# OpenIFEM/OpenIFEM

Hardware: AMD Instinct MI355X
Metric: DoF/s per Newton step (assemble+solve), 3D INS Q2/Q1 (higher is better)
Workload: dtype f64; 1 GPU; 3D channel flow 128x128x128 Q2/Q1, mpi_insim Newton step (plane Poiseuille + seeded 1e-3 perturbation), 128^3 cells per GPU; n_dofs=53070468, cells_per_gpu=2097152, parallelism=dd1, fgmres_iters=1, inner_iters=4, cg_mp_iters=0, cg_sm_iters=2, rccl_nranks=0, comm_transport=none (single rank), halo_neighbors=0

## Files before the change

### __graft_entry__.py

```python
import os
import subprocess
import sys

ROOT = os.path.dirname(os.path.abspath(__file__))
sys.path.insert(0, ROOT)
sys.path.insert(0, os.path.join(ROOT, "tests"))


def build():
    jobs = str(min(8, os.cpu_count() or 1))
    subprocess.check_call(["make", "-C", os.path.join(ROOT, "openifem_amd", "csrc"), "-j", jobs])
    subprocess.check_call(["make", "-C", os.path.join(ROOT, "oracle")])
    import openifem_amd.capi as capi
    L = capi.load()
    missing = [s for s in capi.EXPORTS + capi.EXPORTS_SA_WALL if not hasattr(L, s)]
    if missing:
        raise RuntimeError(f"libifem_hip.so lacks symbols: {missing}")


def smoke():
    import numpy as np
    import openifem_amd.capi as capi
    import orc
    from boxmesh import BoxMesh
    from cases import channel3d_state

    m = BoxMesh([4, 4, 4], (0, 0, 0), (2.0, 0.2, 0.2), kv=2)
    dofs, vals, present, evalp, kw = channel3d_state(m)
    ctx = capi.Context(3, 2, m.vcoords, m.cell_unodes, m.cell_pnodes, m.cell_face_bid, m.n_unodes, m.n_pnodes)
    ctx.set_constraints(0, dofs, None)
    ctx.set_constraints(1, dofs, vals)
    ctx.vec_set(capi.VEC_PRESENT, present)
    ctx.vec_set(capi.VEC_EVAL, evalp)
    P = capi.make_params(**kw)
    ctx.opts.ainv_kind = 3
    ctx.assemble(P, False)
    st = ctx.solve(P, False)
    upd = ctx.vec_get(capi.VEC_UPDATE)
# ... 18 lines not shown
```

### include/ifem_hip_testing.h

```cpp
#ifndef IFEM_HIP_TESTING_H
#define IFEM_HIP_TESTING_H
#include "ifem_hip.h"
#ifdef __cplusplus
extern "C" {
#endif

int ifem_tpp_ilu_probe(ifem_ctx *ctx, int64_t *rowptr, int32_t *col, double *val, const double *x, double *y, int32_t *levels);
int ifem_tpp_override(ifem_ctx *ctx, const double *val);

int ifem_scns_pc_probe(ifem_ctx *ctx, int which, const double *x, double *y);

int ifem_test_restart_fits(ifem_ctx *ctx, int columns);

int ifem_test_mf_uniform(ifem_ctx *ctx, double *h);

int ifem_test_asm_rows(ifem_ctx *ctx, int verbose, int32_t *state);

int ifem_test_uu_vmult_f32col(ifem_ctx *ctx, int dst, int src);

int ifem_test_uu_patch_vmult(ifem_ctx *ctx, int dst, int src);
int ifem_test_uu_patch_info(ifem_ctx *ctx, int64_t out[4]);

enum {
  IFEM_TVK_MDOT = 0, IFEM_TVK_MDOT_SELF, IFEM_TVK_MAXPY, IFEM_TVK_MAXPY_NORM, IFEM_TVK_MDOT_F32, IFEM_TVK_MAXPY_F32, IFEM_TVK_MAXPY_F32_NORM,
  IFEM_TVK_SCALE_STORE_F32, IFEM_TVK_AXPY, IFEM_TVK_AXPBY, IFEM_TVK_SCALE_TO2, IFEM_TVK_DIV, IFEM_TVK_MINMAX, IFEM_TVK_COUNT
};
int ifem_test_vec_kernel(ifem_ctx *ctx, int op, int64_t n, int k, int64_t ld, void *V, const double *coef, double *w, double *out);

int ifem_test_cg_device(ifem_ctx *ctx, int64_t n, const double *a, const double *jac, const double *b, int iters, double *x);

int ifem_test_uu_fused_product(ifem_ctx *ctx, int prec, int mode, int first, double a, double b, const double *x, double *xs, double *r, double *d,
                               int block_cap, int64_t geo[2]);

enum { IFEM_TMG_PAD = 8 };
int ifem_test_mg_transfer(ifem_ctx *ctx, int kind, int64_t n_rows, int64_t n_cols, const int64_t *ptr, const int32_t *col, const double *w,
                          const uint8_t *flag_in, const uint8_t *flag_out, const double *x, double *y);

int ifem_test_mg_lattice_transfer(ifem_ctx *fine, int which, int path, const double *x, double *y, int64_t info[4]);

// ... 20 lines not shown
```

### openifem_amd/capi.py

```python
import ctypes as C
import os

import numpy as np

_HERE = os.path.dirname(os.path.abspath(__file__))
os.environ.setdefault("HSA_ENABLE_IPC_MODE_LEGACY", "0")
LIB_PATH = os.path.join(_HERE, "lib", "libifem_hip.so")

VEC_PRESENT, VEC_EVAL, VEC_FSI_ACC, VEC_UPDATE, VEC_RHS, VEC_INCREMENT, VEC_TMP = range(7)
E_BADPARAM, E_NODEVICE, E_HIP, E_KRYLOV_NOCONV, E_NEWTON_MAXIT, E_COMM = -1, -2, -3, -4, -5, -6
E_NODEVICE_EXIT = 66
AINV_GMRES_BJACOBI, AINV_GMRES_BJACOBI_F32, AINV_SCALAR_GMRES, AINV_GMRES_BJACOBI_MF, AINV_MG = range(5)


class MeshDesc(C.Structure):
    _fields_ = [("dim", C.c_int32), ("kv", C.c_int32), ("n_cells", C.c_int32),
                ("n_unodes_owned", C.c_int32), ("n_unodes_local", C.c_int32),
                ("n_pnodes_owned", C.c_int32), ("n_pnodes_local", C.c_int32),
                ("vcoords", C.c_void_p), ("cell_unodes", C.c_void_p), ("cell_pnodes", C.c_void_p),
                ("cell_face_bid", C.c_void_p)]


class Partition(C.Structure):
    _fields_ = [("rank", C.c_int32), ("nranks", C.c_int32), ("n_neighbors", C.c_int32),
# ... 123 lines not shown
           "ifem_set_cell_fields", "ifem_vec_set", "ifem_vec_get", "ifem_vec_copy", "ifem_vec_zero", "ifem_vec_axpy",
           "ifem_vec_norm2", "ifem_vec_minmax", "ifem_halo_exchange", "ifem_ins_assemble", "ifem_solve",
           "ifem_rhs_norm", "ifem_ins_newton_step", "ifem_system_vmult", "ifem_uu_vmult", "ifem_precond_vmult", "ifem_export_csr",
           "ifem_get_timing", "ifem_set_profiling", "ifem_synchronize", "ifem_set_hanging_constraints", "ifem_set_ainv_kind", "ifem_set_scns_fields", "ifem_update_stress",
           "ifem_scns_assemble", "ifem_scns_solve", "ifem_scns_newton_step", "ifem_imex_assemble", "ifem_imex_solve",
           "ifem_imex_step", "ifem_set_eddy_viscosity", "ifem_default_tuning", "ifem_set_tuning", "ifem_abi_sizeof",
           "ifem_mass_vmult", "ifem_mg_attach", "ifem_mg_depth", "ifem_uu_block_diag",
           "ifem_fsi_set_solid", "ifem_fsi_update_indicator", "ifem_fsi_find_fluid_bc", "ifem_fsi_get_stress",
           "ifem_get_constraints", "ifem_fsi_fluid_at_points", "ifem_comm_stats_get", "ifem_comm_stats_level", "ifem_true_residual", "ifem_tpp_ilu_probe", "ifem_tpp_override", "ifem_scns_pc_probe", "ifem_test_restart_fits",
           "ifem_kprof_begin", "ifem_kprof_end", "ifem_kprof_family_name", "ifem_export_rows", "ifem_export_uu_pattern", "ifem_vcycle_graph_stats", "ifem_inner_restart_length",
           "ifem_uu_stored_bytes", "ifem_test_mf_uniform", "ifem_test_asm_rows", "ifem_test_uu_vmult_f32col",
           "ifem_test_uu_patch_vmult", "ifem_test_uu_patch_info", "ifem_test_vec_kernel", "ifem_test_cg_device",
           "ifem_test_uu_fused_product", "ifem_test_mp_solve", "ifem_test_sm_apply", "ifem_test_b_apply", "ifem_test_sm_solve",
           "ifem_test_mg_transfer", "ifem_test_mg_vec_kernel", "ifem_test_mg_lattice_transfer",
           "ifem_sa_set_wall_points", "ifem_sa_get_wall_distance", "ifem_sa_set_constraints", "ifem_sa_vec_set", "ifem_sa_vec_get",
           "ifem_sa_assemble", "ifem_sa_solve", "ifem_sa_newton_step", "ifem_sa_update_eddy_viscosity", "ifem_sa_export_csr",
           "ifem_scnsex_setup", "ifem_scnsex_assemble_rhs", "ifem_scnsex_solve", "ifem_scnsex_step", "ifem_scnsex_export_csr",
           "ifem_kelly_estimate", "ifem_transfer_solution"]
FACE_BOUNDARY, FACE_EQUAL, FACE_COARSER, FACE_FINER = range(4)

EXPORTS_SA_WALL = ["ifem_sa_set_moving_wall", "ifem_sa_set_shear_velocities", "ifem_sa_update_shear_velocity", "ifem_sa_get_shear_velocity", "ifem_sa_update_moving_wall_distance",
                   "ifem_sa_get_moving_wall", "ifem_sa_update_boundary_condition", "ifem_sa_get_constraints"]
SA_NO_MOVING_WALL = np.finfo(float).max

SM_CG, SM_MG, SM_DIRECT = 0, 1, 2

(TVK_MDOT, TVK_MDOT_SELF, TVK_MAXPY, TVK_MAXPY_NORM, TVK_MDOT_F32, TVK_MAXPY_F32, TVK_MAXPY_F32_NORM, TVK_SCALE_STORE_F32, TVK_AXPY,
 TVK_AXPBY, TVK_SCALE_TO2, TVK_DIV, TVK_MINMAX) = range(13)

(TMG_CHEB_INIT, TMG_CHEB_STEP, TMG_VEC_RECIP, TMG_VEC_ROUGH, TMG_CVT_D2F, TMG_CVT_F2D, TMG_AXPY_F32V, TMG_VC_EXIT, TMG_VC_EXIT_F32,
 TMG_INJECT_NODES, TMG_VC_ENTRY, TMG_VC_ENTRY_F32, TMG_CHEB_INIT_BLOCK_F32) = range(13)
TMG_PAD = 8

ABI_STRUCTS = None

_lib = None


class IfemError(RuntimeError):
    def __init__(self, code, msg):
        super().__init__(f"ifem error {code}: {msg}")
        self.code = code


def load():
    global _lib
# ... 48 lines not shown
    L.ifem_set_ainv_kind.argtypes = [C.c_void_p, C.c_int]
    L.ifem_set_scns_fields.argtypes = [C.c_void_p, C.c_void_p, C.c_void_p, C.c_void_p]
    L.ifem_set_eddy_viscosity.argtypes = [C.c_void_p, C.c_void_p]
    L.ifem_update_stress.argtypes = [C.c_void_p, C.c_double, C.c_void_p]
    L.ifem_scns_assemble.argtypes = [C.c_void_p, C.POINTER(ScnsParams), C.c_int]
    L.ifem_imex_assemble.argtypes = [C.c_void_p, C.POINTER(InsParams), C.c_int, C.c_int]
    L.ifem_imex_solve.argtypes = [C.c_void_p, C.POINTER(InsParams), C.POINTER(SolverOpts), C.c_int, C.POINTER(SolveStats)]
    L.ifem_imex_step.argtypes = [C.c_void_p, C.POINTER(InsParams), C.POINTER(SolverOpts), C.c_int, C.c_int, C.POINTER(SolveStats)]
    L.ifem_scns_solve.argtypes = [C.c_void_p, C.POINTER(SolverOpts), C.c_int, C.POINTER(SolveStats)]
    L.ifem_scns_newton_step.argtypes = [C.c_void_p, C.POINTER(ScnsParams), C.POINTER(SolverOpts), C.c_int, C.c_double,
                                        C.c_int, C.c_void_p]
    L.ifem_default_tuning.argtypes = [C.POINTER(Tuning)]
    L.ifem_set_tuning.argtypes = [C.c_void_p, C.POINTER(Tuning)]
    L.ifem_mg_attach.argtypes = [C.c_void_p, C.c_void_p, C.POINTER(MgTransfer)]
    L.ifem_mg_depth.argtypes = [C.c_void_p]
    L.ifem_comm_stats_get.argtypes = [C.c_void_p, C.c_void_p, C.c_int]
    L.ifem_comm_stats_level.argtypes = [C.c_void_p, C.c_int, C.c_void_p]
    L.ifem_tpp_ilu_probe.argtypes = [C.c_void_p] + [C.c_void_p] * 6
    L.ifem_tpp_override.argtypes = [C.c_void_p, C.c_void_p]
    L.ifem_scns_pc_probe.argtypes = [C.c_void_p, C.c_int, C.c_void_p, C.c_void_p]
    L.ifem_test_restart_fits.argtypes = [C.c_void_p, C.c_int]
    L.ifem_test_mf_uniform.argtypes = [C.c_void_p, C.c_void_p]
    L.ifem_test_asm_rows.argtypes = [C.c_void_p, C.c_int, C.c_void_p]
    L.ifem_test_uu_vmult_f32col.argtypes = [C.c_void_p, C.c_int, C.c_int]
    L.ifem_test_uu_patch_vmult.argtypes = [C.c_void_p, C.c_int, C.c_int]
    L.ifem_test_uu_patch_info.argtypes = [C.c_void_p, C.c_void_p]
    L.ifem_test_vec_kernel.argtypes = [C.c_void_p, C.c_int, C.c_int64, C.c_int, C.c_int64, C.c_void_p, C.c_void_p, C.c_void_p, C.c_void_p]
    L.ifem_test_cg_device.argtypes = [C.c_void_p, C.c_int64, C.c_void_p, C.c_void_p, C.c_void_p, C.c_int, C.c_void_p]
    L.ifem_test_uu_fused_product.argtypes = [C.c_void_p, C.c_int, C.c_int, C.c_int, C.c_double, C.c_double, C.c_void_p, C.c_void_p, C.c_void_p,
                                             C.c_void_p, C.c_int, C.c_void_p]
    L.ifem_test_mp_solve.argtypes = [C.c_void_p, C.POINTER(SolverOpts), C.c_void_p, C.c_void_p, C.c_void_p]
    L.ifem_test_sm_apply.argtypes = [C.c_void_p, C.c_int, C.c_void_p, C.c_void_p, C.c_void_p]
    L.ifem_test_sm_solve.argtypes = [C.c_void_p, C.POINTER(SolverOpts), C.c_void_p, C.c_void_p, C.c_void_p]
    L.ifem_test_b_apply.argtypes = [C.c_void_p, C.c_int, C.c_int, C.c_void_p, C.c_void_p, C.c_void_p]
    L.ifem_test_mg_transfer.argtypes = [C.c_void_p, C.c_int, C.c_int64, C.c_int64] + [C.c_void_p] * 7
    L.ifem_test_mg_lattice_transfer.argtypes = [C.c_void_p, C.c_int, C.c_int, C.c_void_p, C.c_void_p, C.c_void_p]
    L.ifem_test_mg_vec_kernel.argtypes = [C.c_void_p, C.c_int, C.c_int64, C.c_int64] + [C.c_void_p] * 7
    L.ifem_true_residual.argtypes = [C.c_void_p, C.POINTER(C.c_double), C.POINTER(C.c_double)]
    L.ifem_kprof_begin.argtypes = [C.c_void_p]
    L.ifem_kprof_end.argtypes = [C.c_void_p, C.c_void_p, C.c_int32]
    L.ifem_kprof_family_name.argtypes = [C.c_int32]
    L.ifem_kprof_family_name.restype = C.c_char_p
    L.ifem_uu_block_diag.argtypes = [C.c_void_p, C.c_int, C.c_void_p]
    L.ifem_fsi_set_solid.argtypes = [C.c_void_p, C.POINTER(FsiSolid)]
    L.ifem_fsi_update_indicator.argtypes = [C.c_void_p, C.c_void_p, C.POINTER(C.c_int64)]
    L.ifem_fsi_find_fluid_bc.argtypes = [C.c_void_p, C.c_double, C.c_int, C.c_void_p, C.POINTER(FsiStats)]
# ... 294 lines not shown
    def __del__(self):
        try:
            self.close()
        except Exception:
            pass

    def set_tuning(self, **kw):
        t = Tuning()
        self.L.ifem_default_tuning(C.byref(t))
        if getattr(self, "_tuning", None) is not None:
            t = self._tuning
        for k, v in kw.items():
            if not hasattr(t, k):
                raise AttributeError(k)
            setattr(t, k, v)
        self._chk(self.L.ifem_set_tuning(self.h, C.byref(t)))
        self._tuning = t

    def asm_rows_state(self, verbose=False):
        st = C.c_int32(0)
        self._chk(self.L.ifem_test_asm_rows(self.h, int(verbose), C.byref(st)))
        return int(st.value)

    def uu_stored_bytes(self):
        return int(self.L.ifem_uu_stored_bytes(self.h))

    def mf_uniform(self):
        h = np.zeros(3)
        return bool(self._chk(self.L.ifem_test_mf_uniform(self.h, _ptr(h)))), h

    def uu_patch_info(self):
        out = np.zeros(4, np.int64)
        self._chk(self.L.ifem_test_uu_patch_info(self.h, _ptr(out)))
        return bool(out[0]), int(out[1]), int(out[2]), int(out[3])

    def uu_patch_vmult(self, x):
        self.vec_set(VEC_TMP, x)
        self._chk(self.L.ifem_test_uu_patch_vmult(self.h, VEC_UPDATE, VEC_TMP))
        return self.vec_get(VEC_UPDATE)

    def uu_fused_product(self, prec, mode, x, xs=None, r=None, first=0, a=0.0, b=0.0, block_cap=0):
        n = self.dim * self.n_unodes_owned
        x = np.ascontiguousarray(x[:n], float)
        xs = None if mode == 0 else np.array(xs[:n], float)
        r = None if mode == 0 else np.array(r[:n], float)
        d = None if mode == 1 else np.zeros(n)
# ... 376 lines not shown
```

### openifem_amd/csrc/api.hip

```cpp
#include <hip/hip_runtime.h>
#include <chrono>
#include <cmath>
#include <cstdlib>
#include <cstring>
#include <string>
#include <type_traits>
#include <vector>
#include "../../include/ifem_hip_testing.h"
#include "ctx.hpp"
#include "kernels.hpp"
#include "sa_wall_function.hpp"

using namespace ifem;

static thread_local std::string g_err;

#define IFEM_API_BEGIN try {
#define IFEM_API_END                                           \
  }                                                            \
  catch (const ifem::Error &e) { g_err = e.what(); return e.code; } \
  catch (const std::exception &e) { g_err = e.what(); return IFEM_E_HIP; } \
  return IFEM_OK;

namespace ifem {
// ... 1643 lines not shown
  ifem::comm_stats(c, out, false, true);
  IFEM_API_END
}

int ifem_test_restart_fits(ifem_ctx *ctx, int columns) {
  if (!ctx || columns < 0) return IFEM_E_BADPARAM;
  ctx->test_restart_fits = columns;
  return IFEM_OK;
}

int ifem_test_mf_uniform(ifem_ctx *ctx, double *h) {
  if (!ctx) return IFEM_E_BADPARAM;
  if (h) for (int d = 0; d < 3; ++d) h[d] = ctx->mf_uniform ? ctx->mf_h[d] : 0.0;
  return ifem::mf_takes_uniform(ctx) ? 1 : 0;
}

int ifem_test_asm_rows(ifem_ctx *ctx, int verbose, int32_t *state) {
  if (!ctx || !state) return IFEM_E_BADPARAM;
  *state = ctx->rows_state;
  if (verbose && ctx->rows_state < 0) fprintf(stderr, "[ifem] A_uu row owners refused: %s\n", ctx->rows_why ? ctx->rows_why : "?");
  return IFEM_OK;
}

int ifem_inner_restart_length(ifem_ctx *ctx) { return ctx ? ctx->inner_restart_eff : IFEM_E_BADPARAM; }

int ifem_vcycle_graph_stats(ifem_ctx *ctx, uint64_t *captures, uint64_t *launches) {
  IFEM_API_BEGIN
  if (captures) *captures = ctx->vc_graph.captures + ctx->sm_graph.captures + ctx->pa_graph.captures;
  if (launches) *launches = ctx->vc_graph.launches + ctx->sm_graph.launches + ctx->pa_graph.launches;
  IFEM_API_END
}

int ifem_kprof_begin(ifem_ctx *ctx) {
  IFEM_API_BEGIN
  ifem::KProf &k = ifem::kprof_root(ctx);
  k.recs.clear();
  k.used = 0;
  k.depth = 0;
  k.on = true;
  IFEM_API_END
}

int ifem_kprof_end(ifem_ctx *ctx, ifem_kprof_entry *out, int32_t max_entries) {
  int written = 0;
  IFEM_API_BEGIN
  ifem::KProf &k = ifem::kprof_root(ctx);
// ... 45 lines not shown
```

### openifem_amd/csrc/assemble_rows.hip

```cpp
#include <hip/hip_runtime.h>
#include "kernels.hpp"
#include "assemble_common.hpp"
#include "assemble_rows.hpp"

namespace ifem {

typedef double d4 __attribute__((ext_vector_type(4)));
typedef double d2 __attribute__((ext_vector_type(2)));
typedef __attribute__((address_space(1))) double gdouble;
typedef __attribute__((address_space(1))) d2 gd2;

struct RowArgs {
  int64_t n_owners;
  int n[3];
  const int32_t *node_of_lattice;
  const int32_t *cell_at;
  const uint16_t *posUU;
  const int64_t *rp_uu;
  double *v_uu, *rhs;
  const uint8_t *is_c;
  const double *cval;
  const double *pd, *fe;
  const int32_t *pnode_of_lattice;
  int64_t p_off_c, p_off_rhs;
  const Tabs3 *tabs3;
  double ih[3], vol;
  double mu, rho, gamma, inv_dt;
  int use_inhom, imex;
};

struct RowWave {
  static constexpr int IMG = 1128;
  double img[IMG];
  double wq[28];
  double part[4 * 3];
  int64_t rs[8];
  int32_t len[8];
  int32_t nb[125];
  int32_t pcell[32];
  uint8_t cm[128];
  uint16_t pos[27 * 27 + 7];
  uint8_t pa[32];
};

struct RowAcc {
  d4 acc0[9], acc1[9], sac0, sac1;
};

template <int TI, int R0, int NR, int G0, int NG>
__device__ __forceinline__ void node_rows(const RowArgs &A, RowWave &S, const RowAcc &R, const int lane, const bool any_c) {
  constexpr rows::Pair P0 = rows::pair_of(16 * TI + G0 + 4 * R0);
  const int node = S.nb[rows::nb_of_node(P0.nd)];
  if (node < 0) return;
  const int g = lane >> 4, l15 = lane & 15;
  const int64_t rs = S.rs[P0.nd];
  const int len = S.len[P0.nd];
  const int s = int(rs & 1), n = 9 * len;
  const int m = (s + n + 1) / 2;
  d2 *const img2 = reinterpret_cast<d2 *>(S.img);
  for (int i = lane; i < m; i += 64) img2[i] = d2{0, 0};
  wsync2();
  const unsigned rm = any_c ? S.cm[rows::nb_of_node(P0.nd)] : 0u;
  double rh[3] = {0, 0, 0};
  const bool mine = g >= G0 && g < G0 + NG;
#pragma unroll
// ... 67 lines not shown
      else if (j == m - 1 && ((s + n) & 1)) G[2 * j] = v.x;
      else reinterpret_cast<gd2 *>(base)[j] = v;
    }
  }
  const bool inh = any_c && A.use_inhom;
  if (inh) {
#pragma unroll
    for (int c = 0; c < 3; ++c) {
      double v = rh[c];
      v += __shfl_xor(v, 1); v += __shfl_xor(v, 2); v += __shfl_xor(v, 4); v += __shfl_xor(v, 8);
      if (l15 == 0) S.part[g * 3 + c] = v;
    }
    wsync2();
  }
  if (lane < 3) {
    double v = 0;
    if (!((rm >> lane) & 1u)) {
#pragma unroll
      for (int r = R0; r < R0 + NR; ++r)
#pragma unroll
        for (int gg = G0; gg < G0 + NG; ++gg) {
          const int p = 16 * TI + gg + 4 * r;
          const int cell = S.pcell[p];
          if (cell >= 0) v += A.fe[int64_t(cell) * 96 + lane * 27 + S.pa[p]];
        }
    }
    if (inh)
#pragma unroll
      for (int gg = G0; gg < G0 + NG; ++gg) v += S.part[gg * 3 + lane];
    A.rhs[int64_t(3) * node + lane] = v;
  }
  wsync2();
}

template <int TI>
__device__ __forceinline__ void contract(const RowArgs &A, const Tabs3 &T, const RowWave &S, RowAcc &R, const int lane) {
  constexpr int BS = 9;
  const int l15 = lane & 15, g = lane >> 4;
  const int b9_0 = l15 % 9, b3_0 = l15 / 9, b9_1 = (16 + l15) % 9, b3_1 = (16 + l15) / 9;
  const int al = S.pa[16 * TI + l15];
  const int a9 = al % 9, a3 = al / 9;
  const int cell = S.pcell[16 * TI + l15];
  const double *const pd = A.pd + int64_t(cell < 0 ? 0 : cell) * (27 * 12);
  const double wgam = A.gamma * A.rho, rdt = A.rho * A.inv_dt;
  R.sac0 = d4{0, 0, 0, 0}; R.sac1 = d4{0, 0, 0, 0};
#pragma unroll
  for (int e = 0; e < BS; ++e) { R.acc0[e] = d4{0, 0, 0, 0}; R.acc1[e] = d4{0, 0, 0, 0}; }
#pragma unroll 1
  for (int ks = 0; ks < 7; ++ks) {
    const int q = 4 * ks + g;
    const int q3 = q / 9, q9 = (q - q3 * 9) * 9, q4 = q3 * 4;
    const double w = S.wq[q];
    double pq[12];
#pragma unroll
    for (int i = 0; i < 12; ++i) pq[i] = 0.0;
    if (!A.imex) {
      const d2 *src = reinterpret_cast<const d2 *>(pd + (q < 27 ? q : 26) * 12);
#pragma unroll
      for (int i = 0; i < 6; ++i) { const d2 v = src[i]; pq[2 * i] = v.x; pq[2 * i + 1] = v.y; }
    }
    double Na, Nb0, Nb1, ga[3], gb0[3], gb1[3];
    shape_ref4(T, q9, q4, a9, a3, Na, ga);
    shape_ref4(T, q9, q4, b9_0, b3_0, Nb0, gb0);
    shape_ref4(T, q9, q4, b9_1, b3_1, Nb1, gb1);
#pragma unroll
    for (int d = 0; d < 3; ++d) { ga[d] *= A.ih[d]; gb0[d] *= A.ih[d]; gb1[d] *= A.ih[d]; }
    const double wmu = w * A.mu, wg = w * wgam;
#pragma unroll
    for (int e = 0; e < 3; ++e) {
      const double av = pq[e] * Na + wmu * ga[e];
      R.sac0 = __builtin_amdgcn_mfma_f64_16x16x4f64(av, gb0[e], R.sac0, 0, 0, 0);
      R.sac1 = __builtin_amdgcn_mfma_f64_16x16x4f64(av, gb1[e], R.sac1, 0, 0, 0);
    }
#pragma unroll
    for (int c = 0; c < 3; ++c) {
      const double wga = wg * ga[c];
#pragma unroll
      for (int d = 0; d < 3; ++d) {
        R.acc0[c * 3 + d] = __builtin_amdgcn_mfma_f64_16x16x4f64(wga, gb0[d], R.acc0[c * 3 + d], 0, 0, 0);
        R.acc1[c * 3 + d] = __builtin_amdgcn_mfma_f64_16x16x4f64(wga, gb1[d], R.acc1[c * 3 + d], 0, 0, 0);
      }
    }
    if (!A.imex) {
#pragma unroll
      for (int e = 0; e < BS; ++e) {
        const double an = Na * pq[3 + e];
        R.acc0[e] = __builtin_amdgcn_mfma_f64_16x16x4f64(an, Nb0, R.acc0[e], 0, 0, 0);
        R.acc1[e] = __builtin_amdgcn_mfma_f64_16x16x4f64(an, Nb1, R.acc1[e], 0, 0, 0);
      }
    } else {
      const double am = rdt * w * Na;
      R.sac0 = __builtin_amdgcn_mfma_f64_16x16x4f64(am, Nb0, R.sac0, 0, 0, 0);
      R.sac1 = __builtin_amdgcn_mfma_f64_16x16x4f64(am, Nb1, R.sac1, 0, 0, 0);
    }
  }
}

template <int WPB>
__global__ __launch_bounds__(64 * WPB) __attribute__((amdgpu_waves_per_eu(2, 2))) void k_ins_assemble_rows(RowArgs A, Tab1D t1) {
  __shared__ Tabs3 T;
  __shared__ __align__(16) RowWave SW[WPB];
  const int wave = threadIdx.x >> 6, lane = threadIdx.x & 63;
  {
    const double *src = reinterpret_cast<const double *>(A.tabs3);
    double *dst = reinterpret_cast<double *>(&T);
    for (int i = threadIdx.x; i < int(sizeof(Tabs3) / 8); i += 64 * WPB) dst[i] = src[i];
  }
  __syncthreads();
  const int64_t owner = int64_t(blockIdx.x) * WPB + wave;
  if (owner >= A.n_owners) return;
  RowWave &S = SW[wave];
  int ijk[3];
  rows::owner_ijk(owner, A.n, ijk);
  bool cmine = false;
  for (int t = lane; t < 125; t += 64) {
    const int64_t at = rows::nb_point(ijk, A.n, t);
    const int32_t node = at >= 0 ? A.node_of_lattice[at] : -1;
    unsigned mk = 0;
    if (node >= 0 && A.is_c) mk = unsigned(A.is_c[int64_t(3) * node] != 0) | unsigned(A.is_c[int64_t(3) * node + 1] != 0) << 1 | unsigned(A.is_c[int64_t(3) * node + 2] != 0) << 2;
    S.nb[t] = node;
    S.cm[t] = uint8_t(mk);
    const int tx = t % 5 - 2, ty = (t / 5) % 5 - 2, tz = t / 25 - 2;
    if (node >= 0 && (tx | ty | tz) >= 0 && tx < 2 && ty < 2 && tz < 2) {
      const int64_t r0 = A.rp_uu[node];
      S.rs[tx | ty << 1 | tz << 2] = r0;
      S.len[tx | ty << 1 | tz << 2] = int32_t(A.rp_uu[node + 1] - r0);
    }
    cmine = cmine || mk != 0;
  }
  const bool any_c = __any(cmine);
  if (lane < 32) {
    int64_t cell = -1;
    int a = 27;
    if (lane < rows::kPairs) {
      const rows::Pair P = rows::pair_of(lane);
      const int64_t at = rows::row_point(ijk, A.n, P.nd) >= 0 ? rows::pair_cell(ijk, A.n, P) : -1;
      if (at >= 0) { cell = A.cell_at[at]; a = P.a; }
    }
    S.pcell[lane] = int32_t(cell);
    S.pa[lane] = uint8_t(a);
  } else if (lane < 32 + 28) {
    const int q = lane - 32;
    const int qi[3] = {q % 3, (q / 3) % 3, q / 9};
    double wq = A.vol;
#pragma unroll
    for (int d = 0; d < 3; ++d) wq *= t1.w[0] * (qi[d] == 0) + t1.w[1] * (qi[d] == 1) + t1.w[2] * (qi[d] == 2);
    S.wq[q] = q < 27 ? wq : 0.0;
  }
  wsync2();
  for (int i = lane; i < rows::kPairs * 27; i += 64) {
    const int p = i / 27;
    const int cell = S.pcell[p];
    if (cell >= 0) S.pos[i] = A.posUU[(int64_t(cell) * 27 + S.pa[p]) * 27 + (i - p * 27)];
  }
  RowAcc R;
  contract<0>(A, T, S, R, lane);
  node_rows<0, 0, 2, 0, 4>(A, S, R, lane, any_c);
  if (lane == 0) {
    const int64_t pn = A.pnode_of_lattice[owner];
    if (!(A.is_c && A.is_c[A.p_off_c + pn])) {
      double v = 0;
      for (int p = 0; p < 8; ++p) {
        const int cell = S.pcell[p];
        if (cell >= 0) v += A.fe[int64_t(cell) * 96 + 81 + p];
      }
      A.rhs[A.p_off_rhs + pn] = v;
    }
  }
  node_rows<0, 2, 1, 0, 4>(A, S, R, lane, any_c);
  node_rows<0, 3, 1, 0, 4>(A, S, R, lane, any_c);
  contract<1>(A, T, S, R, lane);
  node_rows<1, 0, 1, 0, 4>(A, S, R, lane, any_c);
  node_rows<1, 1, 1, 0, 2>(A, S, R, lane, any_c);
  node_rows<1, 1, 1, 2, 2>(A, S, R, lane, any_c);
  node_rows<1, 2, 1, 0, 2>(A, S, R, lane, any_c);
  node_rows<1, 2, 1, 2, 1>(A, S, R, lane, any_c);
}

__global__ void k_rows_cell_at(int64_t n_cells, const int32_t *__restrict__ cell_unodes, const int32_t *__restrict__ lattice_of_node, int nl0, int nl1, int n0, int n1,
                               int32_t *__restrict__ cell_at) {
  const int64_t c = int64_t(blockIdx.x) * blockDim.x + threadIdx.x;
  if (c >= n_cells) return;
  const int64_t at = lattice_of_node[cell_unodes[c * 27 + 13]];
  const int x = int(at % nl0), y = int((at / nl0) % nl1), z = int(at / (int64_t(nl0) * nl1));
  cell_at[(x >> 1) + int64_t(n0) * ((y >> 1) + int64_t(n1) * (z >> 1))] = int32_t(c);
}

// ... 3 lines not shown
#else
  if (c.dim != 3 || c.kv != 2 || c.nu != 27) return "not 3D Q2 velocity";
  if (c.halo.nranks > 1 || c.nUo != c.nUl) return "several ranks";
  if (c.hang.active || c.hang.n > 0) return "hanging-node lines";
  if (!c.mf_uniform) return "the cells are not one axis-aligned box";
  if (c.want_shat) return "the scalar operator (Shat) is wanted";
  if (c.u_lattice.state < 0) return "the velocity nodes are no full lattice";
  return nullptr;
#endif
}

bool assemble_rows_ensure(ifem_ctx *ctx) {
  if (!u_lattice_ensure(ctx)) return false;
  const ULattice &L = ctx->u_lattice;
  int n[3];
  for (int d = 0; d < 3; ++d) n[d] = (L.n[d] - 1) / 2;
  if (int64_t(n[0]) * n[1] * n[2] != ctx->n_cells) return false;
  if (ctx->rows_cell_at.n != size_t(ctx->n_cells)) {
    ctx->rows_cell_at.alloc(size_t(ctx->n_cells));
    hipLaunchKernelGGL(k_rows_cell_at, dim3(grid_for(ctx->n_cells)), dim3(256), 0, ctx->stream, ctx->n_cells, ctx->cell_unodes.p, L.lattice_of_node.p, L.n[0], L.n[1], n[0], n[1],
                       ctx->rows_cell_at.p);
    IFEM_HIP_CHECK(hipGetLastError());
  }
  return true;
}

void launch_ins_assemble_rows(ifem_ctx *ctx, const AsmArgs &C) {
  constexpr int WPB = 4;
  const ULattice &L = ctx->u_lattice;
  RowArgs A{};
  for (int d = 0; d < 3; ++d) { A.n[d] = (L.n[d] - 1) / 2; A.ih[d] = 1.0 / ctx->mf_h[d]; }
  A.n_owners = rows::n_owners(A.n);
  A.vol = ctx->mf_h[0] * ctx->mf_h[1] * ctx->mf_h[2];
  A.node_of_lattice = L.node_of_lattice.p; A.cell_at = ctx->rows_cell_at.p;
  A.posUU = ctx->posUU.p; A.rp_uu = ctx->Auu.rowptr.p; A.v_uu = ctx->Auu.val.p; A.rhs = C.rhs;
  A.is_c = C.is_c; A.cval = C.cval; A.use_inhom = C.cval ? C.use_inhom : 0;
  A.pd = C.pd; A.fe = C.fe_out; A.tabs3 = ctx->tabs3.p;
  A.pnode_of_lattice = ctx->p_lattice.node_of_lattice.p; A.p_off_c = int64_t(3) * ctx->nUl; A.p_off_rhs = int64_t(3) * ctx->nUo;
  A.mu = C.mu; A.rho = C.rho; A.gamma = C.gamma; A.inv_dt = C.inv_dt; A.imex = C.imex;
  if (!A.pd || !A.fe || !A.tabs3 || !A.cell_at || !A.pnode_of_lattice) throw Error(IFEM_E_BADPARAM, "row-owner assembly before its cell launch");
  Tab1D t;
  tab1d(t, 2);
  hipLaunchKernelGGL((k_ins_assemble_rows<WPB>), dim3(unsigned((A.n_owners + WPB - 1) / WPB)), dim3(64 * WPB), 0, ctx->stream, A, t);
  IFEM_HIP_CHECK(hipGetLastError());
}

}
```

### openifem_amd/csrc/ctx.hpp

```cpp
#pragma once
#include <array>
#include <hip/hip_runtime.h>
#include <cstdint>
#include <cstdio>
#include <stdexcept>
#include <utility>
#include <string>
#include <vector>
#include "../../include/ifem_hip.h"

namespace ifem {

struct Error : std::runtime_error {
  int code;
  Error(int c, const std::string &m) : std::runtime_error(m), code(c) {}
};

#define IFEM_HIP_CHECK(expr)                                                                        \
  do {                                                                                              \
    hipError_t e_ = (expr);                                                                         \
    if (e_ != hipSuccess)                                                                           \
      throw ::ifem::Error(IFEM_E_HIP, std::string(#expr) + ": " + hipGetErrorString(e_) + " at " + \
                                          __FILE__ + ":" + std::to_string(__LINE__));               \
  } while (0)
// ... 524 lines not shown
  bool b2_valid = false;
  ifem::PlanarCsr TppPat;
  ifem::DBuf<double> mf_ycell;
  ifem::DBuf<double> mf_eval;
  ifem::DBuf<double> mf_lift;
  ifem_ins_params mf_params{};
  bool mf_valid = false;
  bool mf_noconv = false;
  double mf_ms_total = 0;
  ifem::F32Copy Auu_f32;
  bool last_spmv_f32 = false;
  ifem::DBuf<double> diagMu;
  ifem::DBuf<double> dinvMu;
  ifem::DBuf<double> bjac;
  ifem::F32Copy bjac_f32;
  ifem::DBuf<uint16_t> posUU, posUP, posPU, posPP;
  ifem::DBuf<int32_t> uu_diag_pos;
  ifem::DBuf<uint16_t> scat3;
  ifem::DBuf<uint8_t> hdr3;
  ifem::DBuf<ifem::Tabs3> tabs3;
  bool hdr3_rows = false;
  ifem::DBuf<int32_t> rows_cell_at;
  ifem::DBuf<double> rows_pd, rows_fe;
  int rows_state = 0;
  const char *rows_why = nullptr;
  ifem::DBuf<uint8_t> is_c[2];
  ifem::DBuf<double> cval[2];
  bool has_c[2] = {false, false};
  ifem::DBuf<double> vec[IFEM_N_VECS];
  ifem::DBuf<double> krylovV, krylovZ, innerV, innerZ, work;
  ifem::DBuf<float> innerVf, innerZf;
  ifem::DBuf<double> scal;
  ifem::DBuf<double> partials;
  double *h_scal = nullptr;
  ifem::Halo halo;
  bool assembled = false;
  bool profile = false;
  ifem_timing timing{};
  hipEvent_t ev0 = nullptr, ev1 = nullptr;
  int tight_first_misses = 0, tight_first_backoff = 0;
  double spmv_uu_ms_total = 0;
  ifem::KProf kprof;
  struct VcGraph {
    hipGraph_t graph = nullptr;
    hipGraphExec_t exec = nullptr;
    std::vector<uint64_t> key;
// ... 94 lines not shown
```

### openifem_amd/csrc/kernels.hpp

```cpp
#pragma once
#include <functional>
#include <vector>
#include "ctx.hpp"
#include "lattice.hpp"

namespace ifem {

void build_pattern(ifem_ctx *ctx, PlanarCsr &M, int bs, int64_t n_rows_owned, int R, const int32_t *d_rows, int C,
                   const int32_t *d_cols, DBuf<uint16_t> &pos);

void ensure_auu_values(ifem_ctx *ctx);
bool ensure_scat3(ifem_ctx *ctx, bool with_rows);
void build_schur_pattern(ifem_ctx *ctx);
void build_schur_pattern_owned(ifem_ctx *ctx);
void build_incidence(ifem_ctx *ctx);
void detect_uniform_cells(ifem_ctx *ctx);
int64_t compact_flagged_rows(ifem_ctx *ctx, const int64_t *flag, int64_t n, DBuf<int32_t> &rows);
void build_mf_cell_split(ifem_ctx *ctx);

enum class AsmMode {
  Rhs,
  Full,
  LevelGeometry,
};
struct AsmArgs;
const char *assemble_rows_refusal(const ifem_ctx &c);
bool assemble_rows_ensure(ifem_ctx *ctx);
void launch_ins_assemble_rows(ifem_ctx *ctx, const AsmArgs &A);
void launch_ins_assemble_ex(ifem_ctx *ctx, const ifem_ins_params *p, int use_nonzero, int imex, AsmMode mode);
template <class Args, class Params>
void fill_cell_args(const ifem_ctx *ctx, const Params *p, int cset, Args &A) {
  A.n_cells = ctx->n_cells; A.nUo = ctx->nUo; A.nUl = ctx->nUl; A.nPo = ctx->nPo;
  A.fe = ctx->d_fe.p;
  A.vcoords = ctx->vcoords.p; A.cell_unodes = ctx->cell_unodes.p; A.cell_pnodes = ctx->cell_pnodes.p;
  A.cell_face_bid = ctx->cell_face_bid.p; A.indicator = ctx->indicator.p;
  A.posUU = ctx->posUU.p; A.posUP = ctx->posUP.p; A.posPU = ctx->posPU.p; A.posPP = ctx->posPP.p;
  A.rp_uu = ctx->Auu.rowptr.p; A.rp_bt = ctx->Bt.rowptr.p; A.rp_b = ctx->B.rowptr.p; A.rp_mp = ctx->Mp.rowptr.p;
  A.v_uu = ctx->Auu.val.p; A.v_bt = ctx->Bt.val.p; A.v_b = ctx->B.val.p; A.rhs = ctx->vec[IFEM_VEC_RHS].p;
  const bool constrained = cset >= 0 && ctx->has_c[cset];
  A.is_c = constrained ? ctx->is_c[cset].p : nullptr;
  A.cval = constrained ? ctx->cval[cset].p : nullptr;
  A.use_inhom = (cset == 1 && constrained) ? 1 : 0;
  A.present = ctx->vec[IFEM_VEC_PRESENT].p;
  A.fsi_acc = ctx->indicator.p ? ctx->vec[IFEM_VEC_FSI_ACC].p : nullptr;
  for (int i = 0; i < 3; ++i) A.g[i] = p->gravity[i];
  A.n_neumann = p->n_neumann;
  for (int i = 0; i < 8; ++i) { A.neumann_id[i] = p->neumann_id[i]; A.neumann_p[i] = p->neumann_p[i]; }
}

void fsi_set_solid(ifem_ctx *ctx, const ifem_fsi_solid *s);
void fsi_update_indicator(ifem_ctx *ctx, int32_t *host_out, int64_t *n_artificial);
// ... 224 lines not shown
```

Measured before the change: 329.6 million DoF/s.

## Precompute constant viscous/grad-div element blocks for row-owner assembly on uniform grids

On a uniform Q2 box the viscous, grad-div and IMEX mass contributions do not depend on the cell, so a small kernel now builds a 27x27x9 constant table once per assembly. The row-owner kernel seeds its MFMA accumulators from this table and keeps only the solution-dependent convection terms in its quadrature loop. Per-cell quadrature data are double-buffered through LDS with a prefetch of the next quadrature slab, and the neighbour, pattern and element-RHS gathers are hoisted into registers before one sync. The cost is an extra small kernel launch and more LDS per wave.

```diff
diff --git a/__graft_entry__.py b/__graft_entry__.py
--- a/__graft_entry__.py
+++ b/__graft_entry__.py
@@ -13,7 +13,7 @@
     subprocess.check_call(["make", "-C", os.path.join(ROOT, "oracle")])
     import openifem_amd.capi as capi
     L = capi.load()
-    missing = [s for s in capi.EXPORTS + capi.EXPORTS_SA_WALL if not hasattr(L, s)]
+    missing = [s for s in capi.EXPORTS + capi.EXPORTS_SA_WALL + capi.EXPORTS_ROWS_CONST if not hasattr(L, s)]
     if missing:
         raise RuntimeError(f"libifem_hip.so lacks symbols: {missing}")
 
diff --git a/include/ifem_hip_testing.h b/include/ifem_hip_testing.h
--- a/include/ifem_hip_testing.h
+++ b/include/ifem_hip_testing.h
@@ -15,6 +15,8 @@
 int ifem_test_mf_uniform(ifem_ctx *ctx, double *h);
 
 int ifem_test_asm_rows(ifem_ctx *ctx, int verbose, int32_t *state);
+
+int ifem_test_rows_const(ifem_ctx *ctx, const ifem_ins_params *p, int imex, double *out );
 
 int ifem_test_uu_vmult_f32col(ifem_ctx *ctx, int dst, int src);
 
diff --git a/openifem_amd/capi.py b/openifem_amd/capi.py
--- a/openifem_amd/capi.py
+++ b/openifem_amd/capi.py
@@ -169,6 +169,7 @@
 EXPORTS_SA_WALL = ["ifem_sa_set_moving_wall", "ifem_sa_set_shear_velocities", "ifem_sa_update_shear_velocity", "ifem_sa_get_shear_velocity", "ifem_sa_update_moving_wall_distance",
                    "ifem_sa_get_moving_wall", "ifem_sa_update_boundary_condition", "ifem_sa_get_constraints"]
 SA_NO_MOVING_WALL = np.finfo(float).max
+EXPORTS_ROWS_CONST = ["ifem_test_rows_const"]
 
 SM_CG, SM_MG, SM_DIRECT = 0, 1, 2
 
@@ -263,6 +264,7 @@
     L.ifem_test_restart_fits.argtypes = [C.c_void_p, C.c_int]
     L.ifem_test_mf_uniform.argtypes = [C.c_void_p, C.c_void_p]
     L.ifem_test_asm_rows.argtypes = [C.c_void_p, C.c_int, C.c_void_p]
+    L.ifem_test_rows_const.argtypes = [C.c_void_p, C.POINTER(InsParams), C.c_int, C.c_void_p]
     L.ifem_test_uu_vmult_f32col.argtypes = [C.c_void_p, C.c_int, C.c_int]
     L.ifem_test_uu_patch_vmult.argtypes = [C.c_void_p, C.c_int, C.c_int]
     L.ifem_test_uu_patch_info.argtypes = [C.c_void_p, C.c_void_p]
@@ -603,6 +605,11 @@
         self._chk(self.L.ifem_test_asm_rows(self.h, int(verbose), C.byref(st)))
         return int(st.value)
 
+    def rows_const(self, params, imex=False):
+        out = np.zeros(27 * 27 * 9)
+        self._chk(self.L.ifem_test_rows_const(self.h, C.byref(params), int(imex), _ptr(out)))
+        return out.reshape(27, 27, 3, 3)
+
     def uu_stored_bytes(self):
         return int(self.L.ifem_uu_stored_bytes(self.h))
 
diff --git a/openifem_amd/csrc/api.hip b/openifem_amd/csrc/api.hip
--- a/openifem_amd/csrc/api.hip
+++ b/openifem_amd/csrc/api.hip
@@ -1689,6 +1689,13 @@
   return IFEM_OK;
 }
 
+int ifem_test_rows_const(ifem_ctx *ctx, const ifem_ins_params *p, int imex, double *out) {
+  IFEM_API_BEGIN
+  if (!p || !out) throw Error(IFEM_E_BADPARAM, "ifem_test_rows_const: null argument");
+  ifem::rows_const_table(ctx, p, imex, out);
+  IFEM_API_END
+}
+
 int ifem_inner_restart_length(ifem_ctx *ctx) { return ctx ? ctx->inner_restart_eff : IFEM_E_BADPARAM; }
 
 int ifem_vcycle_graph_stats(ifem_ctx *ctx, uint64_t *captures, uint64_t *launches) {
diff --git a/openifem_amd/csrc/assemble_rows.hip b/openifem_amd/csrc/assemble_rows.hip
--- a/openifem_amd/csrc/assemble_rows.hip
+++ b/openifem_amd/csrc/assemble_rows.hip
@@ -24,15 +24,19 @@
   const int32_t *pnode_of_lattice;
   int64_t p_off_c, p_off_rhs;
   const Tabs3 *tabs3;
+  const double *k0;
   double ih[3], vol;
   double mu, rho, gamma, inv_dt;
   int use_inhom, imex;
 };
 
-struct RowWave {
+struct alignas(16) RowWave {
   static constexpr int IMG = 1128;
-  double img[IMG];
-  double wq[28];
+  union {
+    double img[IMG];
+    d2 pq[2][8][24];
+  };
+  double fe[27 * 3 + 8];
   double part[4 * 3];
   int64_t rs[8];
   int32_t len[8];
@@ -41,6 +45,7 @@
   uint8_t cm[128];
   uint16_t pos[27 * 27 + 7];
   uint8_t pa[32];
+  uint8_t pcb[32];
 };
 
 struct RowAcc {
@@ -154,7 +159,7 @@
         for (int gg = G0; gg < G0 + NG; ++gg) {
           const int p = 16 * TI + gg + 4 * r;
           const int cell = S.pcell[p];
-          if (cell >= 0) v += A.fe[int64_t(cell) * 96 + lane * 27 + S.pa[p]];
+          if (cell >= 0) v += S.fe[p * 3 + lane];
         }
     }
     if (inh)
@@ -165,71 +170,121 @@
   wsync2();
 }
 
+constexpr int kK0Rows = 28, kK0Cols = 32, kK0 = kK0Rows * 9 * kK0Cols;
+
+__global__ __launch_bounds__(256) void k_rows_const(double *__restrict__ K0, Tab1D t, double ih0, double ih1, double ih2, double vol, double mu, double wgam,
+                                                     double rdt, int imex) {
+  const double ih[3] = {ih0, ih1, ih2};
+  for (int i = blockIdx.x * blockDim.x + threadIdx.x; i < kK0; i += gridDim.x * blockDim.x) {
+    const int b = i % kK0Cols, e = (i / kK0Cols) % 9, a = i / (9 * kK0Cols);
+    const int c = e / 3, d = e - 3 * c;
+    double v = 0.0;
+    if (a < 27 && b < 27) {
+      const int ai[3] = {a % 3, (a / 3) % 3, a / 9}, bi[3] = {b % 3, (b / 3) % 3, b / 9};
+      for (int q = 0; q < 27; ++q) {
+        const int qi[3] = {q % 3, (q / 3) % 3, q / 9};
+        double w = vol;
+        for (int k = 0; k < 3; ++k) w *= t.w[qi[k]];
+        double ga[3], gb[3];
+        const double na2 = t.N[qi[0] * 3 + ai[0]] * t.N[qi[1] * 3 + ai[1]], nb2 = t.N[qi[0] * 3 + bi[0]] * t.N[qi[1] * 3 + bi[1]];
+        const double naz = t.N[qi[2] * 3 + ai[2]], nbz = t.N[qi[2] * 3 + bi[2]];
+        ga[0] = t.dN[qi[0] * 3 + ai[0]] * t.N[qi[1] * 3 + ai[1]] * naz * ih[0];
+        ga[1] = t.N[qi[0] * 3 + ai[0]] * t.dN[qi[1] * 3 + ai[1]] * naz * ih[1];
+        ga[2] = na2 * t.dN[qi[2] * 3 + ai[2]] * ih[2];
+        gb[0] = t.dN[qi[0] * 3 + bi[0]] * t.N[qi[1] * 3 + bi[1]] * nbz * ih[0];
+        gb[1] = t.N[qi[0] * 3 + bi[0]] * t.dN[qi[1] * 3 + bi[1]] * nbz * ih[1];
+        gb[2] = nb2 * t.dN[qi[2] * 3 + bi[2]] * ih[2];
+        double s = (w * wgam) * ga[c] * gb[d];
+        if (c == d) {
+          s += (w * mu) * (ga[0] * gb[0] + ga[1] * gb[1] + ga[2] * gb[2]);
+          if (imex) s += (rdt * w) * (na2 * naz) * (nb2 * nbz);
+        }
+        v += s;
+      }
+    }
+    K0[i] = v;
+  }
+}
+
+static void rows_const_ensure(ifem_ctx *ctx) {
+  if (ctx->rows_k0.n != size_t(kK0)) ctx->rows_k0.alloc(size_t(kK0), "the constant terms of the row-owner assembly");
+}
+
+static void launch_rows_const(ifem_ctx *ctx, const double ih[3], double vol, double mu, double rho, double gamma, double inv_dt, int imex) {
+  Tab1D t;
+  tab1d(t, 2);
+  hipLaunchKernelGGL(k_rows_const, dim3(grid_for(kK0)), dim3(256), 0, ctx->stream, ctx->rows_k0.p, t, ih[0], ih[1], ih[2], vol, mu, gamma * rho, rho * inv_dt, imex);
+  IFEM_HIP_CHECK(hipGetLastError());
+}
+
 template <int TI>
-__device__ __forceinline__ void contract(const RowArgs &A, const Tabs3 &T, const RowWave &S, RowAcc &R, const int lane) {
+__device__ __forceinline__ void contract(const RowArgs &A, const Tabs3 &T, RowWave &S, RowAcc &R, const int lane) {
   constexpr int BS = 9;
   const int l15 = lane & 15, g = lane >> 4;
   const int b9_0 = l15 % 9, b3_0 = l15 / 9, b9_1 = (16 + l15) % 9, b3_1 = (16 + l15) / 9;
   const int al = S.pa[16 * TI + l15];
   const int a9 = al % 9, a3 = al / 9;
-  const int cell = S.pcell[16 * TI + l15];
-  const double *const pd = A.pd + int64_t(cell < 0 ? 0 : cell) * (27 * 12);
-  const double wgam = A.gamma * A.rho, rdt = A.rho * A.inv_dt;
   R.sac0 = d4{0, 0, 0, 0}; R.sac1 = d4{0, 0, 0, 0};
 #pragma unroll
-  for (int e = 0; e < BS; ++e) { R.acc0[e] = d4{0, 0, 0, 0}; R.acc1[e] = d4{0, 0, 0, 0}; }
+  for (int r = 0; r < 4; ++r) {
+    const double *const k = A.k0 + int(S.pa[16 * TI + g + 4 * r]) * (9 * kK0Cols) + l15;
+#pragma unroll
+    for (int e = 0; e < BS; ++e) { R.acc0[e][r] = k[e * kK0Cols]; R.acc1[e][r] = k[e * kK0Cols + 16]; }
+  }
+  if (A.imex) return;
+  const int lslot = lane >> 3, lch = lane & 7;
+  const int lcell = S.pcell[lslot];
+  const d2 *const src = reinterpret_cast<const d2 *>(A.pd + int64_t(lcell < 0 ? 0 : lcell) * (27 * 12)) + 3 * lch;
+  const int myslot = S.pcb[16 * TI + l15];
+  d2 nx[3];
+  auto request = [&](int ks) {
+    const bool on = lcell >= 0 && (ks < 6 || lch < 6);
+#pragma unroll
+    for (int i = 0; i < 3; ++i) nx[i] = on ? src[24 * ks + i] : d2{0, 0};
+  };
+  auto hand_over = [&](int half) {
+    d2 *const dst = &S.pq[half][lslot][3 * lch];
+#pragma unroll
+    for (int i = 0; i < 3; ++i) dst[i] = nx[i];
+    wsync2();
+  };
+  request(0);
+  hand_over(0);
 #pragma unroll 1
   for (int ks = 0; ks < 7; ++ks) {
     const int q = 4 * ks + g;
     const int q3 = q / 9, q9 = (q - q3 * 9) * 9, q4 = q3 * 4;
-    const double w = S.wq[q];
+    if (ks < 6) request(ks + 1);
     double pq[12];
-#pragma unroll
-    for (int i = 0; i < 12; ++i) pq[i] = 0.0;
-    if (!A.imex) {
-      const d2 *src = reinterpret_cast<const d2 *>(pd + (q < 27 ? q : 26) * 12);
-#pragma unroll
-      for (int i = 0; i < 6; ++i) { const d2 v = src[i]; pq[2 * i] = v.x; pq[2 * i + 1] = v.y; }
-    }
-    double Na, Nb0, Nb1, ga[3], gb0[3], gb1[3];
-    shape_ref4(T, q9, q4, a9, a3, Na, ga);
+    {
+      const d2 *const mine = &S.pq[ks & 1][myslot][6 * g];
+#pragma unroll
+      for (int i = 0; i < 6; ++i) { const d2 v = mine[i]; pq[2 * i] = v.x; pq[2 * i + 1] = v.y; }
+    }
+    double Nb0, Nb1, gb0[3], gb1[3];
+    const double Na = T.N2[q9 + a9] * T.Nz[q4 + a3];
     shape_ref4(T, q9, q4, b9_0, b3_0, Nb0, gb0);
     shape_ref4(T, q9, q4, b9_1, b3_1, Nb1, gb1);
 #pragma unroll
-    for (int d = 0; d < 3; ++d) { ga[d] *= A.ih[d]; gb0[d] *= A.ih[d]; gb1[d] *= A.ih[d]; }
-    const double wmu = w * A.mu, wg = w * wgam;
+    for (int d = 0; d < 3; ++d) { gb0[d] *= A.ih[d]; gb1[d] *= A.ih[d]; }
 #pragma unroll
     for (int e = 0; e < 3; ++e) {
-      const double av = pq[e] * Na + wmu * ga[e];
+      const double av = pq[e] * Na;
       R.sac0 = __builtin_amdgcn_mfma_f64_16x16x4f64(av, gb0[e], R.sac0, 0, 0, 0);
       R.sac1 = __builtin_amdgcn_mfma_f64_16x16x4f64(av, gb1[e], R.sac1, 0, 0, 0);
     }
 #pragma unroll
-    for (int c = 0; c < 3; ++c) {
-      const double wga = wg * ga[c];
-#pragma unroll
-      for (int d = 0; d < 3; ++d) {
-        R.acc0[c * 3 + d] = __builtin_amdgcn_mfma_f64_16x16x4f64(wga, gb0[d], R.acc0[c * 3 + d], 0, 0, 0);
-        R.acc1[c * 3 + d] = __builtin_amdgcn_mfma_f64_16x16x4f64(wga, gb1[d], R.acc1[c * 3 + d], 0, 0, 0);
-      }
-    }
-    if (!A.imex) {
-#pragma unroll
-      for (int e = 0; e < BS; ++e) {
-        const double an = Na * pq[3 + e];
-        R.acc0[e] = __builtin_amdgcn_mfma_f64_16x16x4f64(an, Nb0, R.acc0[e], 0, 0, 0);
-        R.acc1[e] = __builtin_amdgcn_mfma_f64_16x16x4f64(an, Nb1, R.acc1[e], 0, 0, 0);
-      }
-    } else {
-      const double am = rdt * w * Na;
-      R.sac0 = __builtin_amdgcn_mfma_f64_16x16x4f64(am, Nb0, R.sac0, 0, 0, 0);
-      R.sac1 = __builtin_amdgcn_mfma_f64_16x16x4f64(am, Nb1, R.sac1, 0, 0, 0);
-    }
+    for (int e = 0; e < BS; ++e) {
+      const double an = Na * pq[3 + e];
+      R.acc0[e] = __builtin_amdgcn_mfma_f64_16x16x4f64(an, Nb0, R.acc0[e], 0, 0, 0);
+      R.acc1[e] = __builtin_amdgcn_mfma_f64_16x16x4f64(an, Nb1, R.acc1[e], 0, 0, 0);
+    }
+    if (ks < 6) hand_over((ks + 1) & 1);
   }
 }
 
 template <int WPB>
-__global__ __launch_bounds__(64 * WPB) __attribute__((amdgpu_waves_per_eu(2, 2))) void k_ins_assemble_rows(RowArgs A, Tab1D t1) {
+__global__ __launch_bounds__(64 * WPB) __attribute__((amdgpu_waves_per_eu(2, 2))) void k_ins_assemble_rows(RowArgs A) {
   __shared__ Tabs3 T;
   __shared__ __align__(16) RowWave SW[WPB];
   const int wave = threadIdx.x >> 6, lane = threadIdx.x & 63;
@@ -244,57 +299,86 @@
   RowWave &S = SW[wave];
   int ijk[3];
   rows::owner_ijk(owner, A.n, ijk);
+  int64_t at[2];
+#pragma unroll
+  for (int u = 0; u < 2; ++u) at[u] = lane + 64 * u < 125 ? rows::nb_point(ijk, A.n, lane + 64 * u) : -1;
+  const rows::Pair P = rows::pair_of(lane < rows::kPairs ? lane : 0);
+  const int64_t cat = lane < rows::kPairs && rows::row_point(ijk, A.n, P.nd) >= 0 ? rows::pair_cell(ijk, A.n, P) : -1;
+  int32_t node[2];
+#pragma unroll
+  for (int u = 0; u < 2; ++u) node[u] = A.node_of_lattice[at[u] < 0 ? 0 : at[u]];
+  int32_t mycell = A.cell_at[cat < 0 ? 0 : cat];
+  const int64_t pn = A.pnode_of_lattice[owner];
+#pragma unroll
+  for (int u = 0; u < 2; ++u) if (at[u] < 0) node[u] = -1;
+  if (cat < 0) mycell = -1;
+  if (lane < 32) {
+    S.pcell[lane] = mycell;
+    S.pa[lane] = uint8_t(mycell >= 0 ? P.a : 27);
+    S.pcb[lane] = uint8_t(lane < rows::kPairs ? P.cb : 0);
+  }
+  uint8_t fl[2][3] = {{0, 0, 0}, {0, 0, 0}};
+  uint8_t pfl = 0;
+  int64_t r0[2], r1[2];
+  if (A.is_c) {
+#pragma unroll
+    for (int u = 0; u < 2; ++u)
+#pragma unroll
+      for (int c = 0; c < 3; ++c) fl[u][c] = A.is_c[int64_t(3) * (node[u] < 0 ? 0 : node[u]) + c];
+    pfl = A.is_c[A.p_off_c + pn];
+  }
+#pragma unroll
+  for (int u = 0; u < 2; ++u) { r0[u] = A.rp_uu[node[u] < 0 ? 0 : node[u]]; r1[u] = A.rp_uu[(node[u] < 0 ? 0 : node[u]) + 1]; }
+  wsync2();
+  constexpr int NPOS = (rows::kPairs * 27 + 63) / 64;
+  uint16_t pv[NPOS];
+#pragma unroll
+  for (int u = 0; u < NPOS; ++u) {
+    const int i = lane + 64 * u < rows::kPairs * 27 ? lane + 64 * u : rows::kPairs * 27 - 1;
+    const int p = i / 27;
+    const int cell = S.pcell[p];
+    pv[u] = A.posUU[(int64_t(cell < 0 ? 0 : cell) * 27 + (cell < 0 ? 0 : S.pa[p])) * 27 + (i - p * 27)];
+  }
+  double fv[2];
+#pragma unroll
+  for (int u = 0; u < 2; ++u) {
+    const int i = lane + 64 * u < 27 * 3 + 8 ? lane + 64 * u : 27 * 3 + 7;
+    const int p = i < 81 ? i / 3 : i - 81;
+    const int cell = S.pcell[p];
+    const double v = A.fe[int64_t(cell < 0 ? 0 : cell) * 96 + (i < 81 ? (i - 3 * p) * 27 + (cell < 0 ? 0 : S.pa[p]) : i)];
+    fv[u] = cell >= 0 ? v : 0.0;
+  }
   bool cmine = false;
-  for (int t = lane; t < 125; t += 64) {
-    const int64_t at = rows::nb_point(ijk, A.n, t);
-    const int32_t node = at >= 0 ? A.node_of_lattice[at] : -1;
-    unsigned mk = 0;
-    if (node >= 0 && A.is_c) mk = unsigned(A.is_c[int64_t(3) * node] != 0) | unsigned(A.is_c[int64_t(3) * node + 1] != 0) << 1 | unsigned(A.is_c[int64_t(3) * node + 2] != 0) << 2;
-    S.nb[t] = node;
+#pragma unroll
+  for (int u = 0; u < 2; ++u) {
+    const int t = lane + 64 * u;
+    if (t >= 125) continue;
+    const unsigned mk = node[u] < 0 ? 0u : unsigned(fl[u][0] != 0) | unsigned(fl[u][1] != 0) << 1 | unsigned(fl[u][2] != 0) << 2;
+    S.nb[t] = node[u];
     S.cm[t] = uint8_t(mk);
     const int tx = t % 5 - 2, ty = (t / 5) % 5 - 2, tz = t / 25 - 2;
-    if (node >= 0 && (tx | ty | tz) >= 0 && tx < 2 && ty < 2 && tz < 2) {
-      const int64_t r0 = A.rp_uu[node];
-      S.rs[tx | ty << 1 | tz << 2] = r0;
-      S.len[tx | ty << 1 | tz << 2] = int32_t(A.rp_uu[node + 1] - r0);
+    if (node[u] >= 0 && (tx | ty | tz) >= 0 && tx < 2 && ty < 2 && tz < 2) {
+      S.rs[tx | ty << 1 | tz << 2] = r0[u];
+      S.len[tx | ty << 1 | tz << 2] = int32_t(r1[u] - r0[u]);
     }
     cmine = cmine || mk != 0;
   }
   const bool any_c = __any(cmine);
-  if (lane < 32) {
-    int64_t cell = -1;
-    int a = 27;
-    if (lane < rows::kPairs) {
-      const rows::Pair P = rows::pair_of(lane);
-      const int64_t at = rows::row_point(ijk, A.n, P.nd) >= 0 ? rows::pair_cell(ijk, A.n, P) : -1;
-      if (at >= 0) { cell = A.cell_at[at]; a = P.a; }
-    }
-    S.pcell[lane] = int32_t(cell);
-    S.pa[lane] = uint8_t(a);
-  } else if (lane < 32 + 28) {
-    const int q = lane - 32;
-    const int qi[3] = {q % 3, (q / 3) % 3, q / 9};
-    double wq = A.vol;
-#pragma unroll
-    for (int d = 0; d < 3; ++d) wq *= t1.w[0] * (qi[d] == 0) + t1.w[1] * (qi[d] == 1) + t1.w[2] * (qi[d] == 2);
-    S.wq[q] = q < 27 ? wq : 0.0;
-  }
-  wsync2();
-  for (int i = lane; i < rows::kPairs * 27; i += 64) {
-    const int p = i / 27;
-    const int cell = S.pcell[p];
-    if (cell >= 0) S.pos[i] = A.posUU[(int64_t(cell) * 27 + S.pa[p]) * 27 + (i - p * 27)];
-  }
+#pragma unroll
+  for (int u = 0; u < NPOS; ++u)
+    if (lane + 64 * u < rows::kPairs * 27) S.pos[lane + 64 * u] = pv[u];
+#pragma unroll
+  for (int u = 0; u < 2; ++u)
+    if (lane + 64 * u < 27 * 3 + 8) S.fe[lane + 64 * u] = fv[u];
   RowAcc R;
   contract<0>(A, T, S, R, lane);
   node_rows<0, 0, 2, 0, 4>(A, S, R, lane, any_c);
   if (lane == 0) {
-    const int64_t pn = A.pnode_of_lattice[owner];
-    if (!(A.is_c && A.is_c[A.p_off_c + pn])) {
+    if (!pfl) {
       double v = 0;
       for (int p = 0; p < 8; ++p) {
         const int cell = S.pcell[p];
-        if (cell >= 0) v += A.fe[int64_t(cell) * 96 + 81 + p];
+        if (cell >= 0) v += S.fe[81 + p];
       }
       A.rhs[A.p_off_rhs + pn] = v;
     }
@@ -344,6 +428,7 @@
                        ctx->rows_cell_at.p);
     IFEM_HIP_CHECK(hipGetLastError());
   }
+  rows_const_ensure(ctx);
   return true;
 }
 
@@ -360,11 +445,23 @@
   A.pd = C.pd; A.fe = C.fe_out; A.tabs3 = ctx->tabs3.p;
   A.pnode_of_lattice = ctx->p_lattice.node_of_lattice.p; A.p_off_c = int64_t(3) * ctx->nUl; A.p_off_rhs = int64_t(3) * ctx->nUo;
   A.mu = C.mu; A.rho = C.rho; A.gamma = C.gamma; A.inv_dt = C.inv_dt; A.imex = C.imex;
-  if (!A.pd || !A.fe || !A.tabs3 || !A.cell_at || !A.pnode_of_lattice) throw Error(IFEM_E_BADPARAM, "row-owner assembly before its cell launch");
-  Tab1D t;
-  tab1d(t, 2);
-  hipLaunchKernelGGL((k_ins_assemble_rows<WPB>), dim3(unsigned((A.n_owners + WPB - 1) / WPB)), dim3(64 * WPB), 0, ctx->stream, A, t);
+  if (!A.pd || !A.fe || !A.tabs3 || !A.cell_at || !A.pnode_of_lattice || !ctx->rows_k0.p) throw Error(IFEM_E_BADPARAM, "row-owner assembly before its cell launch");
+  launch_rows_const(ctx, A.ih, A.vol, A.mu, A.rho, A.gamma, A.inv_dt, A.imex);
+  A.k0 = ctx->rows_k0.p;
+  hipLaunchKernelGGL((k_ins_assemble_rows<WPB>), dim3(unsigned((A.n_owners + WPB - 1) / WPB)), dim3(64 * WPB), 0, ctx->stream, A);
   IFEM_HIP_CHECK(hipGetLastError());
 }
 
-}
+void rows_const_table(ifem_ctx *ctx, const ifem_ins_params *p, int imex, double *out) {
+  if (ctx->dim != 3 || ctx->kv != 2 || !ctx->mf_uniform) throw Error(IFEM_E_BADPARAM, "ifem_test_rows_const: the context is no uniform 3D Q2 box");
+  double ih[3];
+  for (int d = 0; d < 3; ++d) ih[d] = 1.0 / ctx->mf_h[d];
+  rows_const_ensure(ctx);
+  launch_rows_const(ctx, ih, ctx->mf_h[0] * ctx->mf_h[1] * ctx->mf_h[2], p->viscosity, p->rho, p->grad_div, 1.0 / p->dt, imex);
+  const std::vector<double> k = ctx->rows_k0.download(ctx->stream);
+  for (int a = 0; a < 27; ++a)
+    for (int b = 0; b < 27; ++b)
+      for (int e = 0; e < 9; ++e) out[(a * 27 + b) * 9 + e] = k[(a * 9 + e) * kK0Cols + b];
+}
+
+}
diff --git a/openifem_amd/csrc/ctx.hpp b/openifem_amd/csrc/ctx.hpp
--- a/openifem_amd/csrc/ctx.hpp
+++ b/openifem_amd/csrc/ctx.hpp
@@ -570,6 +570,7 @@
   bool hdr3_rows = false;
   ifem::DBuf<int32_t> rows_cell_at;
   ifem::DBuf<double> rows_pd, rows_fe;
+  ifem::DBuf<double> rows_k0;
   int rows_state = 0;
   const char *rows_why = nullptr;
   ifem::DBuf<uint8_t> is_c[2];
diff --git a/openifem_amd/csrc/kernels.hpp b/openifem_amd/csrc/kernels.hpp
--- a/openifem_amd/csrc/kernels.hpp
+++ b/openifem_amd/csrc/kernels.hpp
@@ -27,6 +27,7 @@
 const char *assemble_rows_refusal(const ifem_ctx &c);
 bool assemble_rows_ensure(ifem_ctx *ctx);
 void launch_ins_assemble_rows(ifem_ctx *ctx, const AsmArgs &A);
+void rows_const_table(ifem_ctx *ctx, const ifem_ins_params *p, int imex, double *out);
 void launch_ins_assemble_ex(ifem_ctx *ctx, const ifem_ins_params *p, int use_nonzero, int imex, AsmMode mode);
 template <class Args, class Params>
 void fill_cell_args(const ifem_ctx *ctx, const Params *p, int cset, Args &A) {
```

After: 402.2 million DoF/s (median of 6 runs). +22.1%, better.
